# marksgraham/ddpm-ood

Hardware: AMD Instinct MI355X
Metric: reconstructions/sec (whole node), FashionMNIST 32x32 (higher is better)
Workload: dtype f32 (split-f16 MFMA products, fp32 accumulate)

## Files before the change

### ddpm_ood_amd/csrc/common.h

```cpp
#pragma once
#include <hip/hip_runtime.h>
#include <stdint.h>
#include <stdio.h>
#include <string>

#include "../../include/ddpm_ood_hip.h"

namespace ddpm {

void set_error(const char *fmt, ...);

inline hipStream_t as_stream(ddpm_stream_t s) { return reinterpret_cast<hipStream_t>(s); }

#define DDPM_CHECK_ARG(cond, ...)                \
  do {                                           \
    if (!(cond)) {                               \
      ::ddpm::set_error(__VA_ARGS__);            \
      return DDPM_EINVAL;                        \
    }                                            \
  } while (0)

#define DDPM_CHECK_LAUNCH()                                                    \
  do {                                                                         \
    hipError_t e_ = hipGetLastError();                                         \
    if (e_ != hipSuccess) {                                                    \
      ::ddpm::set_error("%s:%d: %s", __FILE__, __LINE__, hipGetErrorString(e_)); \
      return (int)e_;                                                          \
    }                                                                          \
  } while (0)

constexpr int kWave = 64;

struct Switches {
  int conv_wino44 = 1;
  bool wino44_f16x3 = true;
  int wino44_split = 4;
  int wino_split = 8;
  int wino44_xmap = -1;
  int w44_abl = 0;
  int w44r_serp = 0;
  int w44h_xitem = 1;
  bool up_wino44h = true;
  int down_s2h = 1;
  bool conv1x1_f16x3 = true;
  bool attn_f16x3 = true;
  int d1s_maxpx = 16384;
  int conv_d3s = 1;
  int attn_fa = 1;
  bool conv_splitk = true;
  bool conv_winograd = true;
  bool linear_skinny = true;
  bool conv1x1_dma = true;
  bool gn_fused = true;
  bool attn_waves8 = true;
  bool convin_fast = true;
  bool convout_wave = true;
  long convout_w16_maxwg = -1;
  long convin_blocks_per_cu = 8;
  bool wgrad_f16x3 = true;
  bool prof_shapes = false;
  bool split_f16 = true;
};
const Switches &sw();
unsigned switch_epoch();
inline bool split_f16_on(bool family) { return family && sw().split_f16; }

unsigned *status_word();
__device__ __forceinline__ bool non_finite(float v) { return !(__builtin_fabsf(v) <= 3.402823466e+38f); }

__device__ __forceinline__ void philox_round(uint32_t (&c)[4], uint32_t (&k)[2]) {
  const uint64_t p0 = (uint64_t)0xD2511F53u * c[0], p1 = (uint64_t)0xCD9E8D57u * c[2];
  const uint32_t n0 = (uint32_t)(p1 >> 32) ^ c[1] ^ k[0], n1 = (uint32_t)p1, n2 = (uint32_t)(p0 >> 32) ^ c[3] ^ k[1], n3 = (uint32_t)p0;
  c[0] = n0; c[1] = n1; c[2] = n2; c[3] = n3;
  k[0] += 0x9E3779B9u;
  k[1] += 0xBB67AE85u;
}
__device__ __forceinline__ void philox_normal4(int64_t q, uint64_t stream, uint64_t seed, float (&z)[4]) {
  uint32_t c[4] = {(uint32_t)q, (uint32_t)((uint64_t)q >> 32), (uint32_t)stream, (uint32_t)(stream >> 32)};
  uint32_t k[2] = {(uint32_t)seed, (uint32_t)(seed >> 32)};
#pragma unroll
  for (int r = 0; r < 10; ++r) philox_round(c, k);
#pragma unroll
  for (int h = 0; h < 2; ++h) {
    const float u1 = ((float)c[2 * h] + 1.0f) * 2.3283064365386963e-10f;
    const float u2 = (float)c[2 * h + 1] * 2.3283064365386963e-10f;
    const float rad = sqrtf(-2.0f * logf(u1 < 1e-30f ? 1e-30f : u1));
    float sn, cs;
    sincosf(6.283185307179586f * u2, &sn, &cs);
    z[2 * h] = rad * cs;
    z[2 * h + 1] = rad * sn;
  }
}

extern bool g_prof_on;
void prof_begin(hipStream_t s, const char *kernel, double flops, double bytes);
void prof_end(hipStream_t s);
struct ProfScope {
  hipStream_t s;
  bool on;
  ProfScope(hipStream_t st, const char *kernel, double flops, double bytes) : s(st), on(g_prof_on) {
    if (on) prof_begin(s, kernel, flops, bytes);
  }
  ~ProfScope() {
    if (on) prof_end(s);
  }
};

__device__ __forceinline__ float silu_f(float v) { return v / (1.0f + expf(-v)); }
__device__ __forceinline__ float silu_fast(float v) {
  return v * __builtin_amdgcn_rcpf(1.0f + __builtin_amdgcn_exp2f(-1.44269504088896341f * v));
}

__device__ __forceinline__ float wave_sum(float v) {
#pragma unroll
  for (int o = 32; o > 0; o >>= 1) v += __shfl_xor(v, o, 64);
  return v;
}
template <int CTRL>
__device__ __forceinline__ float dpp_mov0(float v) {
  return __builtin_bit_cast(float, __builtin_amdgcn_update_dpp(0, __builtin_bit_cast(int, v), CTRL, 0xf, 0xf, true));
}
template <int CTRL>
__device__ __forceinline__ void chan_merge_dpp(float &mean, float &m2, float &halfn) {
  const float mo = dpp_mov0<CTRL>(mean), qo = dpp_mov0<CTRL>(m2);
  const float dl = mo - mean;
  m2 = (m2 + qo) + dl * dl * halfn;
  mean = 0.5f * (mean + mo);
  halfn += halfn;
}
__device__ __forceinline__ float wave_sum_dpp_last_lane(float v) {
  v += dpp_mov0<0x111>(v);
  v += dpp_mov0<0x112>(v);
  v += dpp_mov0<0x114>(v);
  v += dpp_mov0<0x118>(v);
  v += dpp_mov0<0x142>(v);
  v += dpp_mov0<0x143>(v);
  return v;
}
__device__ __forceinline__ void group_moments_last_lane(float &mean, float &m2, float cnt, int lanes) {
  float halfn = 0.5f * cnt;
  chan_merge_dpp<0x111>(mean, m2, halfn);
  chan_merge_dpp<0x112>(mean, m2, halfn);
  if (lanes > 4) {
    chan_merge_dpp<0x114>(mean, m2, halfn);
    chan_merge_dpp<0x118>(mean, m2, halfn);
  }
  if (lanes > 16) chan_merge_dpp<0x142>(mean, m2, halfn);
  if (lanes > 32) chan_merge_dpp<0x143>(mean, m2, halfn);
}
__device__ __forceinline__ float wave_max(float v) {
#pragma unroll
  for (int o = 32; o > 0; o >>= 1) v = fmaxf(v, __shfl_xor(v, o, 64));
  return v;
}

typedef _Float16 f16x8 __attribute__((ext_vector_type(8)));

constexpr float kF16LoScale = 32.f;

__device__ __forceinline__ void split_f16x8(const float (&v)[8], f16x8 &hi, f16x8 &lo, f16x8 &hs) {
#pragma unroll
  for (int t = 0; t < 8; ++t) {
    const _Float16 h = (_Float16)v[t];
    hi[t] = h;
    lo[t] = (_Float16)((v[t] - (float)h) * kF16LoScale);
  }
  hs = hi * (_Float16)(1.f / kF16LoScale);
}

#define DDPM_MFMA_F16X3(acc, ah, al, as, bh, bl, bs)                              \
  do {                                                                            \
    (acc) = __builtin_amdgcn_mfma_f32_32x32x16_f16((as), (bl), (acc), 0, 0, 0);   \
    (acc) = __builtin_amdgcn_mfma_f32_32x32x16_f16((al), (bs), (acc), 0, 0, 0);   \
    (acc) = __builtin_amdgcn_mfma_f32_32x32x16_f16((ah), (bh), (acc), 0, 0, 0);   \
  } while (0)

__device__ __forceinline__ float block_sum_256(float v, float *red) {
  v = wave_sum(v);
  const int lane = threadIdx.x & 63, wave = threadIdx.x >> 6;
  __syncthreads();
  if (lane == 0) red[wave] = v;
  __syncthreads();
  return (red[0] + red[1]) + (red[2] + red[3]);
}

int device_cus();
int conv_dispatch(const ddpm_conv_desc &d, hipStream_t s);
size_t conv_scratch_floats(const ddpm_conv_desc &d);
int conv_stats_parts(const ddpm_conv_desc &d);
bool linear_skinny_supported(const ddpm_conv_desc &d);
int launch_linear_skinny(const ddpm_conv_desc &d, hipStream_t s);
bool conv_d3s_supported(const ddpm_conv_desc &d);
int launch_conv_d3s(const ddpm_conv_desc &d, hipStream_t s);
size_t conv_d3s_scratch_floats(const ddpm_conv_desc &d);
int conv_d3s_stats_parts(const ddpm_conv_desc &d);
bool conv_d3s2_supported(const ddpm_conv_desc &d);
int launch_conv_d3s2(const ddpm_conv_desc &d, hipStream_t s);
size_t conv_d3s2_scratch_floats(const ddpm_conv_desc &d);
bool conv_d1s_supported(const ddpm_conv_desc &d);
int launch_conv_d1s(const ddpm_conv_desc &d, hipStream_t s);
size_t conv_d1s_scratch_floats(const ddpm_conv_desc &d);
size_t conv_d3h_weight_halves(int Cout, int Cin);
int launch_pack_conv_d3h_weight(const float *w_raw, uint16_t *dst, int Cout, int Cin, hipStream_t s);
size_t conv_d1s_weight_halves(int Cout, int Cin);
int launch_pack_conv_d1s_weight(const float *w_raw, uint16_t *dst, int Cout, int Cin, int cout_offset, int Cout_total, hipStream_t s);
bool conv_wino44h_supported(const ddpm_conv_desc &d);
int launch_conv_wino44h(const ddpm_conv_desc &d, hipStream_t s);
size_t conv_wino44h_scratch_floats(const ddpm_conv_desc &d);
int conv_wino44h_stats_parts(const ddpm_conv_desc &d);
size_t wino44h_weight_halves(int Cout, int Cin);
int launch_pack_wino44h_weight(const float *w_raw, uint16_t *w_wino44h, int Cout, int Cin, hipStream_t s, int nkd = 1);
bool conv_wino44_supported(const ddpm_conv_desc &d);
int launch_conv_wino44(const ddpm_conv_desc &d, hipStream_t s);
size_t conv_wino44_scratch_floats(const ddpm_conv_desc &d);
size_t wino44_weight_floats(int Cout, int Cin);
bool conv_wino_supported(const ddpm_conv_desc &d);
int launch_conv_wino(const ddpm_conv_desc &d, hipStream_t s);
size_t conv_wino_scratch_floats(const ddpm_conv_desc &d);
int conv_wino_stats_parts(const ddpm_conv_desc &d);
size_t wino_weight_floats(int Cout, int Cin);
int launch_wino_split_reduce(const ddpm_conv_desc &d, int S, long long pstride, int HW, hipStream_t s);
int wino_split_reduce_stats_parts(int HW);
bool conv_s2h_supported(const ddpm_conv_desc &d);
int launch_conv_s2h(const ddpm_conv_desc &d, hipStream_t s);
int conv_s2h_stats_parts(const ddpm_conv_desc &d);
size_t conv_s2h_weight_halves(int Cout, int Cin);
int launch_pack_conv_s2h_weight(const float *w_raw, uint16_t *dst, int Cout, int Cin, hipStream_t s);
bool conv1x1_dma_supported(const ddpm_conv_desc &d);
int launch_conv1x1_dma(const ddpm_conv_desc &d, hipStream_t s);
size_t conv1x1_h_weight_halves(int Cout, int Cin);
int launch_pack_conv1x1_h_weight(const float *w_raw, uint16_t *dst, int Cout, int Cin, int cout_offset, int Cout_total,
                                 hipStream_t s);
bool conv_mfma_supported(const ddpm_conv_desc &d);
int launch_conv_mfma(const ddpm_conv_desc &d, hipStream_t s);
size_t conv_mfma_scratch_floats(const ddpm_conv_desc &d);
size_t packed_conv_weight_floats(int Cout, int Cin, int ksize);
size_t folded_upsample_weight_floats(int Cout, int Cin);
bool conv_direct_supported(const ddpm_conv_desc &d);
int launch_conv_direct(const ddpm_conv_desc &d, hipStream_t s);
int conv_direct_stats_parts(const ddpm_conv_desc &d);
int launch_pack_wino44_weight(const float *w_raw, float *w_wino44, int Cout, int Cin, hipStream_t s, int nkd = 1);
int launch_pack_wino_weight(const float *w_raw, float *w_wino, int Cout, int Cin, hipStream_t s, int nkd = 1);
int launch_fold_upsample_weight(const float *w_raw, float *w_folded, int Cout, int Cin, hipStream_t s);
int launch_pack_conv_weight(const float *w_raw, float *w_packed, int Cout, int Cin, int ksize, int cout_offset,
                            int Cout_total, hipStream_t s, int src_taps = 0, int tap_off = 0);
size_t packed_convT_weight_floats(int Cout, int Cin, int dims);
int launch_pack_convT_weight(const float *w_raw, float *w_packed, int Cin, int Cout, int dims, hipStream_t s);
int launch_conv3d_k4s2_cin1(const float *in, const float *w, const float *bias, float *out, int B, int Cout, int D,
                            int H, int W, int relu, hipStream_t s);
int launch_convT3d_k4s2_cout1(const float *in, const float *w, const float *bias, float *out, int B, int Cin, int D,
                              int H, int W, hipStream_t s);
int launch_convnd_generic(const float *in, const float *w, const float *bias, const float *residual, float *out, int B, int Cin,
                          int Cout, int Di, int Hi, int Wi, int dims, int k, int stride, int pad, int transposed, int relu,
                          hipStream_t s);
int launch_gn_scale_shift(const float *in1, const float *in2, int C1, int C2, const float *gamma, const float *beta,
                          float *scale, float *shift, int B, int HW, int groups, float eps, hipStream_t s);
int launch_gn_finalize(const float *st1, int parts1, int C1, const float *st2, int parts2, int C2, const float *gamma,
                       const float *beta, float *scale, float *shift, int B, int HW, int groups, float eps, hipStream_t s);
int launch_channel_stats(const float *in, float *stats, int B, int C, int HW, hipStream_t s);
int launch_attention(const float *qkv, const float *residual, float *out, int B, int C, int N, int heads, float scale,
                     hipStream_t s, float *scratch = nullptr, size_t scratch_floats = 0, float *stats_out = nullptr);
bool attention_emits_stats(int B, int C, int N, int heads, const float *scratch, size_t scratch_floats);
size_t attention_fa_scratch_floats(int B, int C, int N, int heads);
bool attention_fa_supported(int B, int C, int N, int heads, const float *scratch, size_t scratch_floats);
int launch_attention_fa(const float *qkv, const float *residual, float *out, int B, int C, int N, int heads, float scale,
                        float *scratch, hipStream_t s);
int launch_timestep_embedding(const int64_t *t, const float *freqs, float *out, int B, int dim, hipStream_t s);
int launch_copy_f32(const float *src, float *dst, int64_t n, hipStream_t s);

constexpr int kConvCc = 4;
constexpr int kConvNT = 128;
constexpr int kConvMT = 128;

}
```

### ddpm_ood_amd/csrc/conv_direct.hip

```cpp
#include <stdlib.h>

#include "common.h"

namespace ddpm {

template <int COB>
__global__ __launch_bounds__(256) void conv_direct_kernel(const ddpm_conv_desc a) {
  const int HWo = a.Ho * a.Wo, HWi = a.Hi * a.Wi;
  const int Cin = a.C1 + a.C2;
  const int T = a.ksize * a.ksize;
  const int pad = a.ksize == 3 ? 1 : 0;
  const int s = a.mode == DDPM_CONV_STRIDE2 ? 2 : 1;
  const bool up = a.mode == DDPM_CONV_UPSAMPLE2;
  const int Hv = up ? a.Ho : a.Hi, Wv = up ? a.Wo : a.Wi;

  const int p = blockIdx.x * 256 + threadIdx.x;
  const int n = blockIdx.z;
  const int co0 = blockIdx.y * COB;
  if (p >= HWo) return;
  const int ho = p / a.Wo, wo = p - ho * a.Wo;

  float acc[COB];
#pragma unroll
  for (int j = 0; j < COB; ++j) acc[j] = 0.f;

  for (int ci = 0; ci < Cin; ++ci) {
    const float *plane = (ci < a.C1) ? a.in1 + ((size_t)n * a.C1 + ci) * HWi
                                     : a.in2 + ((size_t)n * a.C2 + (ci - a.C1)) * HWi;
    float sc = 1.f, sh = 0.f;
    if (a.gscale) {
      sc = a.gscale[(size_t)n * Cin + ci];
      sh = a.gshift[(size_t)n * Cin + ci];
    }
    for (int kh = 0; kh < a.ksize; ++kh) {
      for (int kw = 0; kw < a.ksize; ++kw) {
        const int hv = ho * s + kh - pad, wv = wo * s + kw - pad;
        float v = 0.f;
        if (hv >= 0 && hv < Hv && wv >= 0 && wv < Wv) {
          v = up ? plane[(hv >> 1) * a.Wi + (wv >> 1)] : plane[hv * a.Wi + wv];
          if (a.gscale) v = v * sc + sh;
          if (a.act == DDPM_ACT_SILU) v = silu_fast(v);
          if (a.act == DDPM_ACT_RELU) v = fmaxf(v, 0.f);
        }
        const int t = kh * a.ksize + kw;
#pragma unroll
        for (int j = 0; j < COB; ++j) {
          const int co = (co0 + j < a.Cout) ? co0 + j : a.Cout - 1;
          acc[j] = fmaf(v, a.w_raw[((size_t)co * Cin + ci) * T + t], acc[j]);
        }
      }
    }
  }
#pragma unroll
  for (int j = 0; j < COB; ++j) {
    const int co = co0 + j;
    if (co < a.Cout) {
      const size_t idx = ((size_t)n * a.Cout + co) * HWo + p;
      float v = acc[j];
      if (a.bias) v += a.bias[co];
      if (a.chan_add) v += a.chan_add[(size_t)n * a.chan_add_stride + co];
      if (a.residual) v += a.residual[idx];
      if (a.out_act == DDPM_ACT_RELU) v = fmaxf(v, 0.f);
      a.out[idx] = v;
    }
  }
}

constexpr int kSC_CH = 8;

template <int NPOS>
__global__ __launch_bounds__(256) void conv_smallco_kernel(const ddpm_conv_desc a, int TH, int RS, int PS) {
  extern __shared__ __attribute__((aligned(16))) float tile[];
  const int HW = a.Ho * a.Wo;
  const int Cin = a.C1 + a.C2;
  const int tid = threadIdx.x;
  const int n = blockIdx.y;
  const int h0 = blockIdx.x * TH;
  const bool live = tid < TH * a.Wo;
  const int th = live ? tid / a.Wo : 0, tw = live ? tid - th * a.Wo : 0;

  int soff[NPOS];
#pragma unroll
  for (int j = 0; j < NPOS; ++j) {
    const int r = tid + 256 * j;
    soff[j] = -1;
    if (r < PS) {
      const int ir = r / RS, ic = r - ir * RS;
      const int hv = h0 + ir - 1, wv = ic - 1;
      if (hv >= 0 && hv < a.Hi && wv >= 0 && wv < a.Wi) soff[j] = hv * a.Wi + wv;
    }
  }
  float acc[4] = {0.f, 0.f, 0.f, 0.f};
  const int pix = th * RS + tw;

  float pre[NPOS][kSC_CH], psc[kSC_CH], psh[kSC_CH];
  auto fetch = [&](int c0) {
#pragma unroll
    for (int c = 0; c < kSC_CH; ++c) {
      const int ci = c0 + c;
      const bool okc = ci < Cin;
      const float *plane = !okc ? a.in1
                           : (ci < a.C1) ? a.in1 + ((size_t)n * a.C1 + ci) * HW
                                         : a.in2 + ((size_t)n * a.C2 + (ci - a.C1)) * HW;
#pragma unroll
      for (int j = 0; j < NPOS; ++j) pre[j][c] = (okc && soff[j] >= 0) ? plane[soff[j]] : 0.f;
      psc[c] = (okc && a.gscale) ? a.gscale[(size_t)n * Cin + ci] : 1.f;
      psh[c] = (okc && a.gscale) ? a.gshift[(size_t)n * Cin + ci] : 0.f;
    }
  };
  fetch(0);
  for (int c0 = 0; c0 < Cin; c0 += kSC_CH) {
    __syncthreads();
#pragma unroll
    for (int j = 0; j < NPOS; ++j) {
      const int r = tid + 256 * j;
      if (r < PS) {
#pragma unroll
        for (int c = 0; c < kSC_CH; ++c) {
          float v = 0.f;
          if (soff[j] >= 0 && c0 + c < Cin) {
            v = pre[j][c];
            if (a.gscale) v = v * psc[c] + psh[c];
            if (a.act == DDPM_ACT_SILU) v = silu_fast(v);
            if (a.act == DDPM_ACT_RELU) v = fmaxf(v, 0.f);
          }
          tile[c * PS + r] = v;
        }
      }
    }
    __syncthreads();
    if (c0 + kSC_CH < Cin) fetch(c0 + kSC_CH);
#pragma unroll
    for (int c = 0; c < kSC_CH; ++c) {
      const int ci = c0 + c;
      if (ci < Cin) {
        float x[9];
#pragma unroll
        for (int kh = 0; kh < 3; ++kh)
#pragma unroll
          for (int kw = 0; kw < 3; ++kw) x[kh * 3 + kw] = tile[c * PS + pix + kh * RS + kw];
        for (int co = 0; co < a.Cout; ++co) {
          const float *w = a.w_raw + ((size_t)co * Cin + ci) * 9;
#pragma unroll
          for (int t = 0; t < 9; ++t) acc[co] = fmaf(x[t], w[t], acc[co]);
        }
      }
    }
  }
  const int p = (h0 + th) * a.Wo + tw;
  for (int co = 0; co < a.Cout && live; ++co) {
    const size_t idx = ((size_t)n * a.Cout + co) * HW + p;
    float v = acc[co];
    if (a.bias) v += a.bias[co];
    if (a.chan_add) v += a.chan_add[(size_t)n * a.chan_add_stride + co];
    if (a.residual) v += a.residual[idx];
    if (a.out_act == DDPM_ACT_RELU) v = fmaxf(v, 0.f);
    a.out[idx] = v;
  }
}

constexpr int kSW_NJ = 7;
constexpr int kSW_PPL = 4;

template <int NWV>
__global__ __launch_bounds__(64 * NWV) void conv_smallco_wave_kernel(const ddpm_conv_desc a, int TH, int RS, int PS) {
  extern __shared__ __attribute__((aligned(16))) float lds[];
  const int HW = a.Ho * a.Wo;
  const int Cin = a.C1 + a.C2;
  const int tid = threadIdx.x, lane = tid & 63, wave = __builtin_amdgcn_readfirstlane(tid >> 6);
  const int n = blockIdx.y;
  const int h0 = blockIdx.x * TH;
  float *plane_lds = lds + wave * 2 * PS;

  int soff[kSW_NJ];
#pragma unroll
  for (int j = 0; j < kSW_NJ; ++j) {
    const int r = lane + 64 * j;
    soff[j] = -1;
    if (r < PS) {
      const int ir = r / RS, ic = r - ir * RS;
      const int hv = h0 + ir - 1, wv = ic - 1;
      if (hv >= 0 && hv < a.Hi && wv >= 0 && wv < a.Wi) soff[j] = hv * a.Wi + wv;
    }
  }
  int pix[kSW_PPL];
#pragma unroll
  for (int k = 0; k < kSW_PPL; ++k) {
    const int q = lane + 64 * k;
    const int th = q / a.Wo, tw = q - th * a.Wo;
    pix[k] = (q < TH * a.Wo) ? th * RS + tw : 0;
  }
  float acc[kSW_PPL][4];
#pragma unroll
  for (int k = 0; k < kSW_PPL; ++k)
#pragma unroll
    for (int c = 0; c < 4; ++c) acc[k][c] = 0.f;

  float pre[2][kSW_NJ], psc[2] = {1.f, 1.f}, psh[2] = {0.f, 0.f};
  auto fetch = [&](int slot, int ci) {
    const float *plane = (ci < a.C1) ? a.in1 + ((size_t)n * a.C1 + ci) * HW
                                     : a.in2 + ((size_t)n * a.C2 + (ci - a.C1)) * HW;
#pragma unroll
    for (int j = 0; j < kSW_NJ; ++j) pre[slot][j] = soff[j] >= 0 ? plane[soff[j]] : 0.f;
    if (a.gscale) {
      psc[slot] = a.gscale[(size_t)n * Cin + ci];
      psh[slot] = a.gshift[(size_t)n * Cin + ci];
    }
  };
  auto consume = [&](int slot, int ci, int buf) {
    float *pl = plane_lds + buf * PS;
#pragma unroll
    for (int j = 0; j < kSW_NJ; ++j) {
      const int r = lane + 64 * j;
      if (r < PS) {
        float v = 0.f;
        if (soff[j] >= 0) {
          v = pre[slot][j];
          if (a.gscale) v = v * psc[slot] + psh[slot];
          if (a.act == DDPM_ACT_SILU) v = silu_fast(v);
          if (a.act == DDPM_ACT_RELU) v = fmaxf(v, 0.f);
        }
        pl[r] = v;
      }
    }
    if (ci + 2 * NWV < Cin) fetch(slot, ci + 2 * NWV);
    float wreg[4][9];
#pragma unroll
    for (int co = 0; co < 4; ++co) {
      const float *w = a.w_raw + ((size_t)min(co, a.Cout - 1) * Cin + ci) * 9;
#pragma unroll
      for (int t = 0; t < 9; ++t) wreg[co][t] = w[t];
    }
#pragma unroll
    for (int k = 0; k < kSW_PPL; ++k) {
      float x[9];
#pragma unroll
      for (int kh = 0; kh < 3; ++kh)
#pragma unroll
        for (int kw = 0; kw < 3; ++kw) x[kh * 3 + kw] = pl[pix[k] + kh * RS + kw];
#pragma unroll
      for (int co = 0; co < 4; ++co)
        if (co < a.Cout) {
#pragma unroll
          for (int t = 0; t < 9; ++t) acc[k][co] = fmaf(x[t], wreg[co][t], acc[k][co]);
        }
    }
  };
  if (wave < Cin) fetch(0, wave);
  if (wave + NWV < Cin) fetch(1, wave + NWV);
  for (int ci = wave; ci < Cin; ci += 2 * NWV) {
    consume(0, ci, 0);
    if (ci + NWV < Cin) consume(1, ci + NWV, 1);
  }
  float *red = lds + NWV * 2 * PS;
#pragma unroll
  for (int k = 0; k < kSW_PPL; ++k)
#pragma unroll
    for (int c = 0; c < 4; ++c) red[(wave * 256 + lane + 64 * k) * 4 + c] = acc[k][c];
  __syncthreads();
  if (tid < TH * a.Wo) {
    const int th = tid / a.Wo, tw = tid - th * a.Wo;
    const int p = (h0 + th) * a.Wo + tw;
    for (int co = 0; co < a.Cout; ++co) {
      float v = red[(0 * 256 + tid) * 4 + co];
#pragma unroll
      for (int wv = 1; wv < NWV; ++wv) v += red[(wv * 256 + tid) * 4 + co];
      const size_t idx = ((size_t)n * a.Cout + co) * HW + p;
      if (a.bias) v += a.bias[co];
      if (a.chan_add) v += a.chan_add[(size_t)n * a.chan_add_stride + co];
      if (a.residual) v += a.residual[idx];
      if (a.out_act == DDPM_ACT_RELU) v = fmaxf(v, 0.f);
      a.out[idx] = v;
    }
  }
}

template <int CIN>
__global__ __launch_bounds__(256) void conv_smallci_kernel(const ddpm_conv_desc a) {
  const int HW = a.Ho * a.Wo;
  const int p = blockIdx.x * 256 + threadIdx.x;
  const int n = blockIdx.y;
  if (p >= HW) return;
  const int ho = p / a.Wo, wo = p - ho * a.Wo;
  float x[CIN * 9];
#pragma unroll
  for (int ci = 0; ci < CIN; ++ci) {
    const float *plane = a.in1 + ((size_t)n * CIN + ci) * HW;
#pragma unroll
    for (int kh = 0; kh < 3; ++kh)
#pragma unroll
      for (int kw = 0; kw < 3; ++kw) {
        const int hv = ho + kh - 1, wv = wo + kw - 1;
        x[ci * 9 + kh * 3 + kw] = (hv >= 0 && hv < a.Hi && wv >= 0 && wv < a.Wi) ? plane[hv * a.Wi + wv] : 0.f;
      }
  }
  float *dst = a.out + (size_t)n * a.Cout * HW + p;
  const int cpz = (a.Cout + gridDim.z - 1) / gridDim.z, co_end = min(a.Cout, ((int)blockIdx.z + 1) * cpz);
  extern __shared__ float2 wred[];
  const bool emit = a.stats_out != nullptr;
  const int lane = threadIdx.x & 63, wave = threadIdx.x >> 6;
#pragma unroll 4
  for (int co = blockIdx.z * cpz; co < co_end; ++co) {
    const float *w = a.w_raw + (size_t)co * CIN * 9;
    float acc = 0.f;
#pragma unroll
    for (int k = 0; k < CIN * 9; ++k) acc = fmaf(x[k], w[k], acc);
    if (a.bias) acc += a.bias[co];
    dst[(size_t)co * HW] = acc;
    if (emit) {
      const float mean = wave_sum_dpp_last_lane(acc);
      const float mu = __builtin_bit_cast(float, __builtin_amdgcn_readlane(__builtin_bit_cast(int, mean), 63)) * (1.f / 64.f);
      const float dv = acc - mu;
      const float q = wave_sum_dpp_last_lane(dv * dv);
      if (lane == 63) wred[(co - blockIdx.z * cpz) * 4 + wave] = make_float2(mu, q);
    }
  }
  if (emit) {
    __syncthreads();
    const int parts = HW / 256;
    for (int c = threadIdx.x; c < co_end - (int)blockIdx.z * cpz; c += 256) {
      const float2 w0 = wred[c * 4], w1 = wred[c * 4 + 1], w2 = wred[c * 4 + 2], w3 = wred[c * 4 + 3];
      const float m01 = 0.5f * (w0.x + w1.x), d01 = w1.x - w0.x, q01 = (w0.y + w1.y) + d01 * d01 * 32.f;
      const float m23 = 0.5f * (w2.x + w3.x), d23 = w3.x - w2.x, q23 = (w2.y + w3.y) + d23 * d23 * 32.f;
      const float mm = 0.5f * (m01 + m23), dd = m23 - m01, qq = (q01 + q23) + dd * dd * 64.f;
      const int co = blockIdx.z * cpz + c;
      *reinterpret_cast<float2 *>(a.stats_out + (((size_t)n * a.Cout + co) * parts + blockIdx.x) * 2) = make_float2(mm, qq);
    }
  }
}

static bool smallci_supported(const ddpm_conv_desc &d) {
  const bool on = sw().convin_fast;
  return on && d.C2 == 0 && d.C1 >= 1 && d.C1 <= 4 && d.ksize == 3 && d.mode == DDPM_CONV_NORMAL && !d.gscale &&
         d.act == DDPM_ACT_NONE && !d.chan_add && !d.residual && d.out_act == DDPM_ACT_NONE && d.Cout >= 16 &&
         d.Di <= 1 && d.Do <= 1 && d.dims != 3;
}

static int smallci_stats_parts(const ddpm_conv_desc &d) {
  const int HW = d.Ho * d.Wo;
  if (!smallci_supported(d) || HW % 256 || HW / 256 > 8) return 0;
  return HW / 256;
}

static bool smallco_supported(const ddpm_conv_desc &d, int &TH, int &RS, int &PS) {
  if (d.Cout > 4 || d.ksize != 3 || d.mode != DDPM_CONV_NORMAL || d.Wo > 256 || d.Di > 1 || d.Do > 1) return false;
  TH = 0;
  for (int th = 256 / d.Wo; th >= 1; --th)
    if (d.Ho % th == 0) { TH = th; break; }
  if (TH == 0 || 2 * TH * d.Wo < 256) return false;
  RS = d.Wo + 2;
  PS = (TH + 2) * RS;
  return PS <= 512;
}

int launch_conv_direct(const ddpm_conv_desc &d, hipStream_t s) {
  DDPM_CHECK_ARG(d.w_raw != nullptr, "conv_direct: w_raw is NULL");
  DDPM_CHECK_ARG(d.ksize == 1 || d.ksize == 3, "conv_direct: ksize must be 1 or 3");
  DDPM_CHECK_ARG(d.B <= 65535, "conv_direct: batch > 65535");
  const int HWo = d.Ho * d.Wo;
  const double cin = d.C1 + d.C2, taps = d.ksize * d.ksize;
  const int Cin_i = d.C1 + d.C2;
  int TH, RS, PS;
  if (smallco_supported(d, TH, RS, PS)) {
    ProfScope prof(s, "conv3x3_small_cout", 2.0 * d.B * HWo * d.Cout * cin * 9,
                   4.0 * ((double)d.B * cin * HWo + (double)d.B * HWo * d.Cout + d.Cout * cin * 9));
    dim3 grid(d.Ho / TH, d.B);
    const bool wave_ok = sw().convout_wave;
    if (wave_ok && PS <= 64 * kSW_NJ && Cin_i >= 16) {
      const long w16_max = sw().convout_w16_maxwg;
      const long w16_wgs = w16_max >= 0 ? w16_max : 2L * device_cus();
      if ((long)grid.x * grid.y <= w16_wgs && Cin_i >= 64) {
        const size_t lds_w = ((size_t)16 * 2 * PS + 16 * 256 * 4) * sizeof(float);
        static bool attr_done = false;
        if (!attr_done) {
          (void)hipFuncSetAttribute(reinterpret_cast<const void *>(&conv_smallco_wave_kernel<16>), hipFuncAttributeMaxDynamicSharedMemorySize, 160 * 1024);
          attr_done = true;
        }
        hipLaunchKernelGGL(conv_smallco_wave_kernel<16>, grid, dim3(1024), lds_w, s, d, TH, RS, PS);
        DDPM_CHECK_LAUNCH();
        return 0;
      }
      const size_t lds_w = ((size_t)4 * 2 * PS + 4 * 256 * 4) * sizeof(float);
      hipLaunchKernelGGL(conv_smallco_wave_kernel<4>, grid, dim3(256), lds_w, s, d, TH, RS, PS);
      DDPM_CHECK_LAUNCH();
      return 0;
    }
    const size_t lds = (size_t)kSC_CH * PS * sizeof(float);
    if (PS <= 256)
      hipLaunchKernelGGL(conv_smallco_kernel<1>, grid, dim3(256), lds, s, d, TH, RS, PS);
    else
      hipLaunchKernelGGL(conv_smallco_kernel<2>, grid, dim3(256), lds, s, d, TH, RS, PS);
    DDPM_CHECK_LAUNCH();
    return 0;
  }
  if (smallci_supported(d)) {
    ProfScope prof(s, "conv3x3_small_cin", 2.0 * d.B * HWo * d.Cout * cin * 9,
                   4.0 * ((double)d.B * cin * HWo + (double)d.B * HWo * d.Cout + d.Cout * cin * 9));
    const long blocks = (long)((HWo + 255) / 256) * d.B;
    int zs = 1;
    const long zblk = sw().convin_blocks_per_cu;
    while (zs < 8 && blocks * zs * 2 <= device_cus() * zblk && d.Cout / (zs * 2) >= 16) zs *= 2;
    dim3 grid((HWo + 255) / 256, d.B, zs);
    ddpm_conv_desc dk = d;
    if (smallci_stats_parts(d) == 0) dk.stats_out = nullptr;
    const size_t lds = dk.stats_out ? (size_t)((d.Cout + zs - 1) / zs) * 4 * sizeof(float2) : 0;
    switch (d.C1) {
      case 1: hipLaunchKernelGGL(conv_smallci_kernel<1>, grid, dim3(256), lds, s, dk); break;
      case 2: hipLaunchKernelGGL(conv_smallci_kernel<2>, grid, dim3(256), lds, s, dk); break;
      case 3: hipLaunchKernelGGL(conv_smallci_kernel<3>, grid, dim3(256), lds, s, dk); break;
      default: hipLaunchKernelGGL(conv_smallci_kernel<4>, grid, dim3(256), lds, s, dk); break;
    }
    DDPM_CHECK_LAUNCH();
    return 0;
  }
  ProfScope prof(s, "conv_direct", 2.0 * d.B * HWo * d.Cout * cin * taps,
                 4.0 * ((double)d.B * cin * d.Hi * d.Wi + (double)d.B * HWo * d.Cout * (d.residual ? 2 : 1) +
                        d.Cout * cin * taps));
  if (d.Cout <= 4) {
    dim3 grid((HWo + 255) / 256, d.Cout, d.B);
    hipLaunchKernelGGL(conv_direct_kernel<1>, grid, dim3(256), 0, s, d);
  } else {
    dim3 grid((HWo + 255) / 256, (d.Cout + 7) / 8, d.B);
    hipLaunchKernelGGL(conv_direct_kernel<8>, grid, dim3(256), 0, s, d);
  }
  DDPM_CHECK_LAUNCH();
  return 0;
}

bool conv_direct_supported(const ddpm_conv_desc &) { return true; }

int conv_direct_stats_parts(const ddpm_conv_desc &d) {
  int TH, RS, PS;
  return d.mode == DDPM_CONV_NORMAL && !smallco_supported(d, TH, RS, PS) ? smallci_stats_parts(d) : 0;
}

}
```

Baseline: 1112.

## Add 4-pixel-per-thread quad kernels for small-Cin and small-Cout 3x3 convs

Result: no change. 1120 (median of 6 runs) (+0.7%).

```diff
diff --git a/ddpm_ood_amd/csrc/common.h b/ddpm_ood_amd/csrc/common.h
--- a/ddpm_ood_amd/csrc/common.h
+++ b/ddpm_ood_amd/csrc/common.h
@@ -135,6 +135,13 @@
   v += dpp_mov0<0x118>(v);
   v += dpp_mov0<0x142>(v);
   v += dpp_mov0<0x143>(v);
+  return v;
+}
+__device__ __forceinline__ float row_sum_dpp_all_lanes(float v) {
+  v += dpp_mov0<0xB1>(v);
+  v += dpp_mov0<0x4E>(v);
+  v += dpp_mov0<0x141>(v);
+  v += dpp_mov0<0x140>(v);
   return v;
 }
 __device__ __forceinline__ void group_moments_last_lane(float &mean, float &m2, float cnt, int lanes) {
diff --git a/ddpm_ood_amd/csrc/conv_direct.hip b/ddpm_ood_amd/csrc/conv_direct.hip
--- a/ddpm_ood_amd/csrc/conv_direct.hip
+++ b/ddpm_ood_amd/csrc/conv_direct.hip
@@ -275,6 +275,144 @@
   }
 }
 
+typedef float f32x4 __attribute__((ext_vector_type(4)));
+typedef const float __attribute__((address_space(4))) *cfloat_p;
+__device__ __forceinline__ cfloat_p as_const(const float *p) { return (cfloat_p) reinterpret_cast<uintptr_t>(p); }
+
+template <int NQ, int CO>
+__global__ __launch_bounds__(256) void conv_smallco_quad_kernel(const ddpm_conv_desc a, int TH) {
+  extern __shared__ __attribute__((aligned(16))) float lds[];
+  constexpr int NS = NQ + 1;
+  const int W = a.Wo, H = a.Ho, HW = H * W, QW = W >> 2, RS = W + 4;
+  const int PS = (TH + 2) * RS + 4;
+  const int Cin = a.C1 + a.C2;
+  const int tid = threadIdx.x, lane = tid & 63, wave = __builtin_amdgcn_readfirstlane(tid >> 6);
+  const int n = blockIdx.y;
+  const int h0 = blockIdx.x * TH;
+  float *pl = lds + wave * PS;
+
+  for (int i = lane; i < (PS >> 2); i += 64) reinterpret_cast<f32x4 *>(pl)[i] = f32x4{0.f, 0.f, 0.f, 0.f};
+  const int r0 = max(h0 - 1, 0), r1 = min(h0 + TH + 1, H);
+  const int nst = (r1 - r0) * QW;
+  int goff[NS], loff[NS];
+#pragma unroll
+  for (int j = 0; j < NS; ++j) {
+    const int sq = lane + 64 * j;
+    goff[j] = -1;
+    loff[j] = 0;
+    if (sq < nst) {
+      const int sr = sq / QW, sc = sq - sr * QW, hv = r0 + sr;
+      goff[j] = hv * W + 4 * sc;
+      loff[j] = (hv - h0 + 1) * RS + 4 + 4 * sc;
+    }
+  }
+  int woff[NQ];
+#pragma unroll
+  for (int k = 0; k < NQ; ++k) {
+    const int q = lane + 64 * k, qr = q / QW;
+    woff[k] = qr * RS + 4 * (q - qr * QW);
+  }
+  float acc[NQ][CO][4];
+#pragma unroll
+  for (int k = 0; k < NQ; ++k)
+#pragma unroll
+    for (int co = 0; co < CO; ++co)
+#pragma unroll
+      for (int p = 0; p < 4; ++p) acc[k][co][p] = 0.f;
+
+  f32x4 pre[2][NS];
+  float psc[2] = {1.f, 1.f}, psh[2] = {0.f, 0.f};
+  auto fetch = [&](int slot, int ci) {
+    const float *plane = (ci < a.C1) ? a.in1 + ((size_t)n * a.C1 + ci) * HW
+                                     : a.in2 + ((size_t)n * a.C2 + (ci - a.C1)) * HW;
+#pragma unroll
+    for (int j = 0; j < NS; ++j)
+      if (j * 64 < nst)
+        pre[slot][j] = goff[j] >= 0 ? *reinterpret_cast<const f32x4 *>(plane + goff[j]) : f32x4{0.f, 0.f, 0.f, 0.f};
+    if (a.gscale) {
+      psc[slot] = a.gscale[(size_t)n * Cin + ci];
+      psh[slot] = a.gshift[(size_t)n * Cin + ci];
+    }
+  };
+  auto consume = [&](int slot, int ci) {
+#pragma unroll
+    for (int j = 0; j < NS; ++j)
+      if (j * 64 < nst && goff[j] >= 0) {
+        f32x4 v4 = pre[slot][j];
+#pragma unroll
+        for (int e = 0; e < 4; ++e) {
+          float v = v4[e];
+          if (a.gscale) v = v * psc[slot] + psh[slot];
+          if (a.act == DDPM_ACT_SILU) v = silu_fast(v);
+          if (a.act == DDPM_ACT_RELU) v = fmaxf(v, 0.f);
+          v4[e] = v;
+        }
+        *reinterpret_cast<f32x4 *>(pl + loff[j]) = v4;
+      }
+    asm volatile("" ::: "memory");
+    if (ci + 8 < Cin) fetch(slot, ci + 8);
+    float wreg[CO][9];
+#pragma unroll
+    for (int co = 0; co < CO; ++co) {
+      const cfloat_p w = as_const(a.w_raw) + ((size_t)co * Cin + ci) * 9;
+#pragma unroll
+      for (int t = 0; t < 9; ++t) wreg[co][t] = w[t];
+    }
+#pragma unroll
+    for (int k = 0; k < NQ; ++k) {
+      float x[3][6];
+#pragma unroll
+      for (int kh = 0; kh < 3; ++kh) {
+        const float *row = pl + woff[k] + kh * RS;
+        const f32x4 m = *reinterpret_cast<const f32x4 *>(row + 4);
+        x[kh][0] = row[3];
+        x[kh][1] = m[0], x[kh][2] = m[1], x[kh][3] = m[2], x[kh][4] = m[3];
+        x[kh][5] = row[8];
+      }
+#pragma unroll
+      for (int co = 0; co < CO; ++co)
+#pragma unroll
+        for (int p = 0; p < 4; ++p)
+#pragma unroll
+          for (int t = 0; t < 9; ++t) acc[k][co][p] = fmaf(x[t / 3][p + t % 3], wreg[co][t], acc[k][co][p]);
+    }
+    asm volatile("" ::: "memory");
+  };
+  if (wave < Cin) fetch(0, wave);
+  if (wave + 4 < Cin) fetch(1, wave + 4);
+  for (int ci = wave; ci < Cin; ci += 8) {
+    consume(0, ci);
+    if (ci + 4 < Cin) consume(1, ci + 4);
+  }
+  __syncthreads();
+  f32x4 *red = reinterpret_cast<f32x4 *>(lds);
+#pragma unroll
+  for (int k = 0; k < NQ; ++k)
+#pragma unroll
+    for (int co = 0; co < CO; ++co)
+      red[(wave * CO + co) * (64 * NQ) + lane + 64 * k] = f32x4{acc[k][co][0], acc[k][co][1], acc[k][co][2], acc[k][co][3]};
+  __syncthreads();
+  for (int q = tid; q < 64 * NQ; q += 256) {
+    const int qr = q / QW, qc = q - qr * QW;
+    const int p = (h0 + qr) * W + 4 * qc;
+#pragma unroll
+    for (int co = 0; co < CO; ++co) {
+      f32x4 v = red[co * (64 * NQ) + q];
+#pragma unroll
+      for (int wv = 1; wv < 4; ++wv) v += red[(wv * CO + co) * (64 * NQ) + q];
+      const size_t idx = ((size_t)n * CO + co) * HW + p;
+      if (a.bias) v += a.bias[co];
+      if (a.chan_add) v += a.chan_add[(size_t)n * a.chan_add_stride + co];
+      if (a.residual) v += *reinterpret_cast<const f32x4 *>(a.residual + idx);
+      if (a.out_act == DDPM_ACT_RELU) {
+#pragma unroll
+        for (int e = 0; e < 4; ++e) v[e] = fmaxf(v[e], 0.f);
+      }
+      *reinterpret_cast<f32x4 *>(a.out + idx) = v;
+    }
+  }
+}
+
 template <int CIN>
 __global__ __launch_bounds__(256) void conv_smallci_kernel(const ddpm_conv_desc a) {
   const int HW = a.Ho * a.Wo;
@@ -329,6 +467,70 @@
   }
 }
 
+template <int CIN>
+__global__ __launch_bounds__(64) void conv_smallci_quad_kernel(const ddpm_conv_desc a) {
+  const int W = a.Wo, HW = a.Ho * W, QW = W >> 2;
+  const int q = blockIdx.x * 64 + threadIdx.x;
+  const int n = blockIdx.y;
+  if (4 * q >= HW) return;
+  const int ho = q / QW, wo = 4 * (q - ho * QW);
+  float x[CIN][3][6];
+#pragma unroll
+  for (int ci = 0; ci < CIN; ++ci) {
+    const float *plane = a.in1 + ((size_t)n * CIN + ci) * HW;
+#pragma unroll
+    for (int kh = 0; kh < 3; ++kh) {
+      const int hv = ho + kh - 1;
+      const bool okr = hv >= 0 && hv < a.Hi;
+      const float *row = plane + (okr ? hv : 0) * W + wo;
+      const f32x4 m = okr ? *reinterpret_cast<const f32x4 *>(row) : f32x4{0.f, 0.f, 0.f, 0.f};
+      x[ci][kh][0] = (okr && wo > 0) ? row[-1] : 0.f;
+      x[ci][kh][1] = m[0], x[ci][kh][2] = m[1], x[ci][kh][3] = m[2], x[ci][kh][4] = m[3];
+      x[ci][kh][5] = (okr && wo + 4 < W) ? row[4] : 0.f;
+    }
+  }
+  float *dst = a.out + (size_t)n * a.Cout * HW + 4 * q;
+  const int cpz = (a.Cout + gridDim.z - 1) / gridDim.z, co_end = min(a.Cout, ((int)blockIdx.z + 1) * cpz);
+  const bool emit = a.stats_out != nullptr;
+  const int parts = HW >> 8;
+  const cfloat_p wts = as_const(a.w_raw), bias = as_const(a.bias);
+  float wn[CIN * 9], bn = 0.f;
+  auto wload = [&](int co) {
+#pragma unroll
+    for (int k = 0; k < CIN * 9; ++k) wn[k] = wts[(size_t)co * CIN * 9 + k];
+    if (a.bias) bn = bias[co];
+  };
+  if ((int)blockIdx.z * cpz < co_end) wload(blockIdx.z * cpz);
+  for (int co = blockIdx.z * cpz; co < co_end; ++co) {
+    float w[CIN * 9];
+#pragma unroll
+    for (int k = 0; k < CIN * 9; ++k) w[k] = wn[k];
+    const float b = bn;
+    wload(min(co + 1, co_end - 1));
+    float acc[4] = {0.f, 0.f, 0.f, 0.f};
+#pragma unroll
+    for (int p = 0; p < 4; ++p)
+#pragma unroll
+      for (int k = 0; k < CIN * 9; ++k) acc[p] = fmaf(x[k / 9][(k % 9) / 3][p + k % 3], w[k], acc[p]);
+    if (a.bias) {
+#pragma unroll
+      for (int p = 0; p < 4; ++p) acc[p] += b;
+    }
+    *reinterpret_cast<f32x4 *>(dst + (size_t)co * HW) = f32x4{acc[0], acc[1], acc[2], acc[3]};
+    if (emit) {
+      const float mu = row_sum_dpp_all_lanes((acc[0] + acc[1]) + (acc[2] + acc[3])) * (1.f / 64.f);
+      const float d0 = acc[0] - mu, d1 = acc[1] - mu, d2 = acc[2] - mu, d3 = acc[3] - mu;
+      float mean = mu, m2 = row_sum_dpp_all_lanes((d0 * d0 + d1 * d1) + (d2 * d2 + d3 * d3)), halfn = 32.f;
+      chan_merge_dpp<0x142>(mean, m2, halfn);
+      chan_merge_dpp<0x143>(mean, m2, halfn);
+      if (threadIdx.x == 63)
+        *reinterpret_cast<float2 *>(a.stats_out + (((size_t)n * a.Cout + co) * parts + blockIdx.x) * 2) = make_float2(mean, m2);
+    }
+  }
+}
+
+static bool aligned16(const void *p) { return (reinterpret_cast<uintptr_t>(p) & 15) == 0; }
+
 static bool smallci_supported(const ddpm_conv_desc &d) {
   const bool on = sw().convin_fast;
   return on && d.C2 == 0 && d.C1 >= 1 && d.C1 <= 4 && d.ksize == 3 && d.mode == DDPM_CONV_NORMAL && !d.gscale &&
@@ -351,6 +553,33 @@
   RS = d.Wo + 2;
   PS = (TH + 2) * RS;
   return PS <= 512;
+}
+
+static bool smallci_quad_ok(const ddpm_conv_desc &d) { return d.Wo % 4 == 0 && aligned16(d.in1) && aligned16(d.out); }
+
+static int smallco_quad_rows(const ddpm_conv_desc &d, long min_wgs) {
+  if (d.Wo % 4 || d.Wo > 128 || d.Cout < 1 || d.Cout > 4) return 0;
+  if (!aligned16(d.in1) || (d.C2 && !aligned16(d.in2)) || !aligned16(d.out) || (d.residual && !aligned16(d.residual))) return 0;
+  const int QW = d.Wo / 4;
+  int best = 0;
+  for (int nq = 4; nq >= 1; nq >>= 1) {
+    if ((64 * nq) % QW) continue;
+    const int th = 64 * nq / QW;
+    if (th < 2 || th > d.Ho || d.Ho % th) continue;
+    best = th;
+    if ((long)(d.Ho / th) * d.B >= min_wgs) break;
+  }
+  return best;
+}
+
+template <int NQ>
+static void launch_smallco_quad(const ddpm_conv_desc &d, int TH, dim3 grid, size_t lds, hipStream_t s) {
+  switch (d.Cout) {
+    case 1: hipLaunchKernelGGL((conv_smallco_quad_kernel<NQ, 1>), grid, dim3(256), lds, s, d, TH); break;
+    case 2: hipLaunchKernelGGL((conv_smallco_quad_kernel<NQ, 2>), grid, dim3(256), lds, s, d, TH); break;
+    case 3: hipLaunchKernelGGL((conv_smallco_quad_kernel<NQ, 3>), grid, dim3(256), lds, s, d, TH); break;
+    default: hipLaunchKernelGGL((conv_smallco_quad_kernel<NQ, 4>), grid, dim3(256), lds, s, d, TH); break;
+  }
 }
 
 int launch_conv_direct(const ddpm_conv_desc &d, hipStream_t s) {
@@ -380,6 +609,18 @@
         DDPM_CHECK_LAUNCH();
         return 0;
       }
+      if (const int qth = smallco_quad_rows(d, 4L * device_cus())) {
+        const int nq = qth * (d.Wo / 4) / 64;
+        const size_t planes = (size_t)4 * ((qth + 2) * (d.Wo + 4) + 4) * sizeof(float);
+        const size_t red = (size_t)4 * d.Cout * 64 * nq * 4 * sizeof(float);
+        const size_t lds_q = planes > red ? planes : red;
+        const dim3 qgrid(d.Ho / qth, d.B);
+        if (nq == 4) launch_smallco_quad<4>(d, qth, qgrid, lds_q, s);
+        else if (nq == 2) launch_smallco_quad<2>(d, qth, qgrid, lds_q, s);
+        else launch_smallco_quad<1>(d, qth, qgrid, lds_q, s);
+        DDPM_CHECK_LAUNCH();
+        return 0;
+      }
       const size_t lds_w = ((size_t)4 * 2 * PS + 4 * 256 * 4) * sizeof(float);
       hipLaunchKernelGGL(conv_smallco_wave_kernel<4>, grid, dim3(256), lds_w, s, d, TH, RS, PS);
       DDPM_CHECK_LAUNCH();
@@ -399,10 +640,22 @@
     const long blocks = (long)((HWo + 255) / 256) * d.B;
     int zs = 1;
     const long zblk = sw().convin_blocks_per_cu;
-    while (zs < 8 && blocks * zs * 2 <= device_cus() * zblk && d.Cout / (zs * 2) >= 16) zs *= 2;
+    const bool quads = smallci_quad_ok(d);
+    const long wpb = quads ? 4 : 1;
+    while (zs < 8 && blocks * zs * 2 <= device_cus() * zblk * wpb && d.Cout / (zs * 2) >= 16) zs *= 2;
     dim3 grid((HWo + 255) / 256, d.B, zs);
     ddpm_conv_desc dk = d;
     if (smallci_stats_parts(d) == 0) dk.stats_out = nullptr;
+    if (quads) {
+      switch (d.C1) {
+        case 1: hipLaunchKernelGGL(conv_smallci_quad_kernel<1>, grid, dim3(64), 0, s, dk); break;
+        case 2: hipLaunchKernelGGL(conv_smallci_quad_kernel<2>, grid, dim3(64), 0, s, dk); break;
+        case 3: hipLaunchKernelGGL(conv_smallci_quad_kernel<3>, grid, dim3(64), 0, s, dk); break;
+        default: hipLaunchKernelGGL(conv_smallci_quad_kernel<4>, grid, dim3(64), 0, s, dk); break;
+      }
+      DDPM_CHECK_LAUNCH();
+      return 0;
+    }
     const size_t lds = dk.stats_out ? (size_t)((d.Cout + zs - 1) / zs) * 4 * sizeof(float2) : 0;
     switch (d.C1) {
       case 1: hipLaunchKernelGGL(conv_smallci_kernel<1>, grid, dim3(256), lds, s, dk); break;
```
